# cszheng-ioa/Sixty-years-of-frequency-domain-monaural-speech-enhancement

Hardware: AMD Instinct MI355X
Metric: utterances/sec, 16 kHz 4 s clips, DCCRN decode (STFT->network->iSTFT) (higher is better)
Workload: dtype f32; 1 GPU; BASELINE configs[2]: DCCRN complex-mask, compressed input (0.5/2.0), 16 kHz x 4 s clips, batch 256 per MI355X, utterance-sharded; batch_per_gpu=256, global_batch=256, clip_samples=64000, parallelism=utterance shard x1 + RCCL gather to rank 0

## Files before the change

sixty-years-of-frequency-domain-monaural-speech-enhancement_amd/csrc/gemmconv.h:

```cpp
#pragma once
#include <hip/hip_runtime.h>
#include <vector>

namespace se {

constexpr int GC_MAX_TAPS = 16;
constexpr int GC_MAX_ROWS = 8;
constexpr int GC_MAX_KCP = 48;
constexpr int GC_TAB_KOFF = GC_MAX_ROWS + 2 * GC_MAX_TAPS;
constexpr int gc_kcp_max(int BM) { return 32; }
constexpr int gc_bld_max(int BM) { return (BM >= 128 || BM <= 32) ? 9 : 13; }
constexpr int gc_blocks_per_cu(int BM) { return BM <= 32 ? 6 : 3; }

enum Act : int { ACT_NONE = 0, ACT_PRELU = 1, ACT_ELU = 2, ACT_SOFTPLUS = 3, ACT_SIGMOID = 4, ACT_TANH = 5, ACT_RELU = 6 };
enum Epi : int {
    EPI_ACT = 0,
    EPI_LSTM = 1,
    EPI_GLU = 2,
    EPI_ADD = 3,
    EPI_MUL = 4,
    EPI_CMB = 5,
};

constexpr int GC_THIN_NT = 8;
// ... 28 lines not shown
    int si, so, po;
    int ntaps, nrows, dtmin, Wp;
    int CI_C, KC, KCp, nchunks;
    int act, epi;
    int n_ttiles, n_mtiles, Z;
    int dbg;
    int first_step;
    int gru;
    unsigned long long* timing;
    const unsigned* desc4;
    int t_base;
    int tb_soft;
    int pw4;
    int causal;
    const int* tlen;
    int qt2, qq_off, Qt;
    int pair, po2, fo_lim;
    short tdf[GC_MAX_TAPS], tdt[GC_MAX_TAPS];
    int nbuf;
    int trim;
    const unsigned* desc;
    const int* tab;
    float* stats;
    long st_b, st_c, st_f;
    float* cstats;
    long cs_b, cs_f;
    float* fz;
    long fz_b, fz_c, fz_f, fz_im;
    long fz_s;
    const float* nrm0;
    const float* nrm1;
    int flat_upr;
    int flat_units;
};
constexpr int GC_NRM_MAXC = 128;
constexpr int GC_FLAT_NRM_ROWS = 2;

struct GCGeom {
    int* tab = nullptr;
    unsigned* desc = nullptr;
    unsigned* desc4 = nullptr;
};
struct GCTail {
    int BN = 0, Wp = 0;
    GCGeom g;
};

struct GCSmallGeom {
    int dfmin = 0, dfmax = 0, dtmin = 0, dtmax = 0;
};

struct GCPlan {
    GCParams p{};
    int BM = 128, BN = 128;
    int lookback = 0;
    double flop_scale = 1.0;
    float* dA = nullptr;
    float* dWs = nullptr;
    unsigned* dDesc = nullptr;
    unsigned* dDesc4 = nullptr;
    GCSmallGeom small;
    bool tail_split = false;
    GCTail tail[3];
    GCTail qt2;
    GCTail flat[2];
    int flat_uw = 0;
    int qt2_nrows = 0, qt2_qoff = 0;
// ... 4 lines not shown
    float* dPostScale = nullptr;
    float* dPostShift = nullptr;
};

struct TapSpec {
    int ntaps = 0;
    int df[GC_MAX_TAPS];
    int dt[GC_MAX_TAPS];
};

GCPlan gc_make_plan(int M, int Cin, const TapSpec& taps, const std::vector<float>& w_logical,
                    const std::vector<float>& bias, const std::vector<float>& slope, int act, int epi,
                    int si, int so, int po, int tout_hint, int z = 1, int C0split = -1);
void gc_free_plan(GCPlan& pl);

void gc_register_overread_range(const void* lo, size_t bytes);
void gc_unregister_overread_range(const void* lo);

bool gc_stats_supported(const GCPlan& pl);
bool gc_nrm_supported(const GCPlan& pl);
void gc_launch(const GCPlan& pl, GCParams p, hipStream_t stream);
bool gc_launch_thin_pair(const GCParams& p0, const GCParams& p1, hipStream_t stream);

enum GCFamily : int { GC_FAM_TILE = 0, GC_FAM_THIN = 1, GC_FAM_THIN_PAIR = 2, GC_FAM_DIRECT = 3, GC_FAM_DIRECT_LDS = 4 };
struct GCLaunchRec {
    int family = GC_FAM_TILE;
    int BM = 0, BN = 0;
    int flat_upr = 0, upt = 0;
    int flat_rows = 0;
    int qt2 = 0, nrm = 0, res = 0, trim = 0, stats = 0, ragged = 0;
    int flat_nrm_refused = 0;
    long nblk = 0;
    int epi = 0, gru = 0;
};
void gc_set_launch_log(std::vector<GCLaunchRec>* log);
int gc_flat_rows_spanned(int B, int upr, int upt);

}
```

sixty-years-of-frequency-domain-monaural-speech-enhancement_amd/csrc/gemmconv.hip:

```cpp
#include "gemmconv.h"
#include "common.h"
#include "fastmath.h"
#include <algorithm>
#include <cmath>
#include <cstring>
#include <mutex>
#include <type_traits>

namespace se {

typedef float floatx16 __attribute__((ext_vector_type(16)));
typedef float floatx4 __attribute__((ext_vector_type(4)));

template <int N, typename F>
__device__ __forceinline__ void static_for(F&& f) {
    if constexpr (N > 0) {
        static_for<N - 1>(f);
        f(std::integral_constant<int, N - 1>{});
    }
}

__device__ __forceinline__ float fsig_(float x) { return fm_sigmoid(x); }
__device__ __forceinline__ float ftanh_(float x) { return fm_tanh(x); }
__device__ __forceinline__ float act_apply(float v, int act, float slope) {
// ... 252 lines not shown
            const int f = q * p.si + tabl[tabl[GC_MAX_ROWS + kr_ - nk_cil * p.ntaps]];
            nk_ok = kr_ < p.KC && f >= 0 && f < p.Fin;
        }
        pb_cil = tid / p.nrows;
    }

    unsigned aoff[A_IT];
    static_for<A_IT>([&](auto I) {
        constexpr int i = decltype(I)::value;
        int idx = tid + i * 256;
        if (idx >= nA4) idx = nA4 - 1;
        aoff[i] = 4u * (unsigned)((idx / (BM / 4)) * p.Mp + (idx % (BM / 4)) * 4);
    });
    unsigned boff[NB];
    unsigned vbits = 0;
    unsigned fullbits = 0;

    floatx16 acc[TM][TN];
#pragma unroll
    for (int i = 0; i < TM; ++i)
#pragma unroll
        for (int j = 0; j < TN; ++j)
#pragma unroll
            for (int r = 0; r < 16; ++r) acc[i][j][r] = 0.f;

    const int wm = wave / WN, wn = (WN == 4 && BN >= 256) ? ((wave + ttile) & 3) : wave % WN;
    constexpr int WNT = WN >= 2 ? WN / 2 : 1;
    const int wq = (qt2 && WN >= 2) ? wn / WNT : 0;
    const int wt = (qt2 && WN >= 2) ? wn % WNT : wn;
    const int am = wm * (TM * 32) + l31;
    const int bn = FLAT ? wn * (TN * UW) + l31 : wq * p.qq_off + wt * (TN * 32) + l31;
    const int jact = FLAT ? max(0, min(TN, p.flat_units - u0 - wn * TN))
                          : (q + wq >= p.Q) ? 0 : max(0, min(TN, (p.Tout - t0 - wt * (TN * 32) + 31) >> 5));

    int gchunk = 0;
    int buf = 0;

#define GC_MAKE_DESC(LIM)                                                                          \
    {                                                                                              \
        const int lim_ = (LIM);                                                                    \
        vbits = 0;                                                                                 \
         \
         \
         \
        unsigned dsc_[NB];                                                                         \
        {                                                                                          \
            const unsigned* __restrict__ dp_ = (pw4 ? p.desc4 : p.desc) + tid;                     \
            static_for<NB>([&](auto E) {                                                           \
                constexpr int e = decltype(E)::value;                                              \
                dsc_[e] = dp_[256 * e];                                                            \
            });                                                                                    \
        }                                                                                          \
        static_for<NB>([&](auto E) {                                                               \
            constexpr int e = decltype(E)::value;                                                  \
            const unsigned d_ = dsc_[e];                                                           \
            const int w = d_ & 0xfff, r = (d_ >> 12) & 0xf, cil = (d_ >> 16) & 0x7fff;             \
            const bool staged = (d_ >> 31) != 0;                                                   \
            const int f = q * p.si + tabl[staged ? r : 0];                                         \
             \
            const int uk_ = FLAT ? min(w / UW, UPT - 1) : 0;                                       \
            const int t = FLAT ? utab[4 * uk_ + 1] + p.dtmin + (w - uk_ * UW) : t0 + p.dtmin + w;  \
            const bool uok_ = !FLAT || utab[4 * uk_ + 2] != 0;                                     \
            const unsigned ub_ = (FLAT && uok_) ? (unsigned)utab[4 * uk_] * sb32 : 0u;             \
            const int fc = f < 0 ? 0 : (f >= p.Fin ? p.Fin - 1 : f);                               \
            const int tc = t < 0 ? 0 : (t >= p.Tin ? p.Tin - 1 : t);                               \
            const int cc = cil < lim_ ? cil : lim_ - 1;                                            \
// ... 115 lines not shown
        GC_WAIT_CHUNK();
        GC_TRIM_TAIL(buf);
        GC_T(3);
        __syncthreads();
        GC_T(4);

        for (int c = 0; c < nch; ++c) {
            if constexpr (RES) {
                if (c > 0 && buf == nbuf) {
                    __syncthreads();
                    for (int c2 = c; c2 < min(nch, c + nbuf); ++c2) {
                        if (c2 + 1 == nch && tail != p.CI_C) GC_MAKE_DESC(tail);
                        GC_LOAD_CHUNK(c2, c2 - c);
                    }
                    GC_WAIT_CHUNK();
                    __syncthreads();
                    buf = 0;
                }
            }
            if (!RES && c + 1 < nch && !(p.dbg & 1)) {
                if (__builtin_expect(c + 2 == nch && tail != p.CI_C, 0)) GC_MAKE_DESC(tail);
                GC_LOAD_CHUNK(c + 1, buf ^ 1);
            }
            GC_T(1);
            const float* Ab = As + buf * As_sz + hi * BM + am;
            const float* Bb = Bs + buf * Bs_sz + bn;
            const floatx4* nkb = nrmK + buf * (NRMB * KCP_MAX) + hi;
            int nkd[FLAT && NRM ? TN : 1];
            if constexpr (FLAT && NRM) {
#pragma unroll
                for (int j = 0; j < TN; ++j) nkd[j] = utab[4 * min(wn * TN + j, UPT - 1)] * KCP_MAX;
            }
            const int npair = p.KCp >> 1;
#define GC_FETCH(KP, AR, BR)                                                                       \
    {                                                                                              \
        int o_;                                                                                    \
        if constexpr (KOFF_REGS) o_ = koffv[(KP) < NPAIR ? (KP) : NPAIR - 1];                      \
        else o_ = koff_lds[2 * (KP) + hi];                                                         \
        _Pragma("unroll") for (int i = 0; i < TM; ++i) AR[i] = Ab[(2 * (KP)) * BM + i * 32];       \
        _Pragma("unroll") for (int j = 0; j < JN; ++j) BR[j] = Bb[o_ + j * UW];                    \
        if constexpr (NRM && !FLAT) {                                                              \
            const floatx4 pr_ = nkb[2 * (KP)];                                                     \
            _Pragma("unroll") for (int j = 0; j < JN; ++j) {                                       \
                const float t_ = fmaf(BR[j], pr_[0], pr_[1]);                                      \
                BR[j] = fmaf(fminf(t_, 0.f), pr_[2], t_);                                          \
            }                                                                                      \
        }                                                                                          \
        if constexpr (NRM && FLAT) {                                                               \
            _Pragma("unroll") for (int j = 0; j < JN; ++j) {                                       \
                const floatx4 pr_ = nkb[2 * (KP) + nkd[j]];                                        \
                const float t_ = fmaf(BR[j], pr_[0], pr_[1]);                                      \
                BR[j] = fmaf(fminf(t_, 0.f), pr_[2], t_);                                          \
            }                                                                                      \
        }                                                                                          \
    }
#define GC_MMA(AR, BR)                                                                             \
    _Pragma("unroll") for (int i = 0; i < TM; ++i)                                                 \
        _Pragma("unroll") for (int j = 0; j < JN; ++j)                                             \
            acc[i][j] = __builtin_amdgcn_mfma_f32_32x32x2f32(AR[i], BR[j], acc[i][j], 0, 0, 0);
            auto mma_chunk = [&](auto JN_) {
                constexpr int JN = decltype(JN_)::value;
                float ax[TM], bx[JN], ay[TM], by[JN];
                GC_FETCH(0, ax, bx);
                static_for<NPAIR / 2>([&](auto KP2) {
                    constexpr int kp = 2 * decltype(KP2)::value;
                    int np_ = npair;
                    asm volatile("" : "+s"(np_));
                    if (kp < np_) {
                        constexpr int NDS = (TM + 1) / 2 + (JN + 1) / 2 + (NRM ? (FLAT ? JN : 1) : 0);
                        GC_FETCH(kp + 1, ay, by);
                        __builtin_amdgcn_sched_group_barrier(0x100, NDS, 0);
                        GC_MMA(ax, bx);
                        __builtin_amdgcn_sched_group_barrier(0x008, TM * JN, 0);
                        if constexpr (NRM) __builtin_amdgcn_sched_group_barrier(0x002, 3 * JN, 0);
                        GC_FETCH(kp + 2, ax, bx);
                        __builtin_amdgcn_sched_group_barrier(0x100, NDS, 0);
                        GC_MMA(ay, by);
                        __builtin_amdgcn_sched_group_barrier(0x008, TM * JN, 0);
                        if constexpr (NRM) __builtin_amdgcn_sched_group_barrier(0x002, 3 * JN, 0);
                    }
                });
            };
            if (!(p.dbg & 4)) {
                if (jact == 1 && TN == 2) mma_chunk(std::integral_constant<int, 1>{});
                else if (jact >= 1) mma_chunk(std::integral_constant<int, TN>{});
            }
#undef GC_FETCH
#undef GC_MMA
            GC_T(2);
            if constexpr (RES) {
                buf += 1;
            } else {
                GC_WAIT_CHUNK();
                GC_TRIM_TAIL(buf ^ 1);
                GC_T(3);
                __syncthreads();
                GC_T(4);
                buf ^= 1;
            }
        }
        if constexpr (RES) __syncthreads();
// ... 557 lines not shown
                    v = act_apply(v, p.act, p.slope ? p.slope[j] : 0.f);
                    if (p.pair) {
                        const int cls = (2 * j) / p.pair, fo2 = (q0 + qq) * p.so + (cls ? p.po2 : p.po);
                        if (fo2 < p.fo_lim) dst[(long)(fo2 - fo) * p.d_f + (long)(j - cls * (p.pair >> 1)) * p.d_c + t] = v;
                    } else {
                        dst[(long)j * p.d_c + t] = v;
                    }
                }
            }
            continue;
        }
#pragma unroll
        for (int m = 0; m < MM; ++m) {
            if (m < p.M) {
                float v = acc[qq][m] + (bias ? bias[m] : 0.f);
                v = act_apply(v, p.act, p.slope ? p.slope[m] : 0.f);
                if (EPI == EPI_ADD) v += res[(long)m * p.x_c + t];
                if (EPI == EPI_MUL) v *= res[(long)m * p.x_c + t];
                if (EPI == EPI_ACT && p.pair) {
                    const int cls = m / p.pair, fo2 = (q0 + qq) * p.so + (cls ? p.po2 : p.po);
                    if (fo2 < p.fo_lim) dst[(long)(fo2 - fo) * p.d_f + (long)(m - cls * p.pair) * p.d_c + t] = v;
                    continue;
                }
                dst[(long)m * p.d_c + t] = v;
            }
        }
    }
}

template <int EPI, int NT>
__device__ __forceinline__ void gc_thin_body(const GCParams& p, const int blk) {
    constexpr int RB = 8, KG = 32, UN = 8;
    __shared__ float part[KG][RB][NT + 1];
    __shared__ int s_df[GC_MAX_TAPS], s_dt[GC_MAX_TAPS];
    const int tid = threadIdx.x, mi = tid & (RB - 1), kg = tid / RB;
#pragma unroll
    for (int j = 0; j < GC_MAX_TAPS; ++j)
        if (tid == j) {
            s_df[j] = p.tdf[j];
            s_dt[j] = p.tdt[j];
        }
    __syncthreads();
    const int nm = (p.M + RB - 1) / RB;
    const int mt = blk % nm;
    const int rest = blk / nm;
    const int q = rest % p.Q, b = rest / p.Q;
    const int m = mt * RB + mi, t0 = p.t_base, n = p.Tout - p.t_base;
    const int ntaps = p.ntaps, Ktot = (p.C0 + p.C1) * ntaps;
    const int nch0 = p.C0 > 0 ? (p.C0 + p.CI_C - 1) / p.CI_C : 0;
    float acc[NT];
#pragma unroll
    for (int t = 0; t < NT; ++t) acc[t] = 0.f;
    for (int k0 = kg; k0 < Ktot; k0 += KG * UN) {
        float w[UN], xv[UN][NT];
#pragma unroll
        for (int u = 0; u < UN; ++u) {
            const int kk = k0 + u * KG;
            const bool kok = kk < Ktot;
            const int kc = kok ? kk : 0;
            const int ci = kc / ntaps, j = kc - ci * ntaps;
            const bool seg = ci >= p.C0;
            const int cs = seg ? ci - p.C0 : ci;
            const int chunk = (seg ? nch0 : 0) + cs / p.CI_C, cil = cs % p.CI_C;
            const float wv = p.A[((long)chunk * p.KCp + cil * ntaps + j) * p.Mp + m];
            const int f = q * p.si + s_df[j];
            const bool fok = kok && f >= 0 && f < p.Fin;
            const int fc = fok ? f : 0;
            const float* __restrict__ src = seg ? p.src1 + (long)b * p.s1_b + (long)cs * p.s1_c + (long)fc * p.s1_f
                                                : p.src0 + (long)b * p.s0_b + (long)cs * p.s0_c + (long)fc * p.s0_f;
            const int tb = t0 + s_dt[j];
            w[u] = fok ? wv : 0.f;
#pragma unroll
            for (int t = 0; t < NT; ++t) {
                const int ti = tb + t;
                const bool ok = t < n && ti >= 0 && ti < p.Tin;
                const float x = src[ok ? ti : 0];
                xv[u][t] = ok ? x : 0.f;
            }
        }
#pragma unroll
        for (int u = 0; u < UN; ++u)
#pragma unroll
            for (int t = 0; t < NT; ++t) acc[t] = fmaf(w[u], xv[u][t], acc[t]);
    }
#pragma unroll
    for (int t = 0; t < NT; ++t) part[kg][mi][t] = acc[t];
    __syncthreads();
    const bool fold = tid < RB * NT;
    const int r = tid & (RB - 1), t = (tid / RB) & (NT - 1);
    float tot = 0.f;
    if (fold) {
#pragma unroll
        for (int g = 0; g < KG; ++g) tot += part[g][r][t];
    }
    __syncthreads();
    if (fold) part[0][r][t] = tot;
    __syncthreads();
// ... 54 lines not shown
__global__ __launch_bounds__(256) void gc_thin_pair_kernel(const GCThinPair a) {
    const int cls = (int)blockIdx.x >= a.nblk0 ? 1 : 0;
    gc_thin_body<EPI, NT>(a.p[cls], (int)blockIdx.x - (cls ? a.nblk0 : 0));
}
template <int EPI>
static void gc_thin_launch_n(const GCParams& p, dim3 grid, int n, hipStream_t stream) {
    if (n <= 1) hipLaunchKernelGGL((gc_thin_kernel<EPI, 1>), grid, dim3(256), 0, stream, p);
    else if (n <= 2) hipLaunchKernelGGL((gc_thin_kernel<EPI, 2>), grid, dim3(256), 0, stream, p);
    else if (n <= 4) hipLaunchKernelGGL((gc_thin_kernel<EPI, 4>), grid, dim3(256), 0, stream, p);
    else hipLaunchKernelGGL((gc_thin_kernel<EPI, 8>), grid, dim3(256), 0, stream, p);
}
static thread_local std::vector<GCLaunchRec>* g_launch_log = nullptr;
static thread_local int g_flat_nrm_refused = 0;
void gc_set_launch_log(std::vector<GCLaunchRec>* log) { g_launch_log = log; }
static void gc_log_launch(int family, const GCParams& p, long nblk, int BM = 0, int BN = 0, bool res = false) {
    if (!g_launch_log) return;
    GCLaunchRec r;
    r.family = family;
    r.BM = BM;
    r.BN = BN;
    r.flat_upr = p.flat_upr;
    r.upt = p.flat_upr ? BN / 32 : 0;
    r.flat_rows = p.flat_upr ? gc_flat_rows_spanned(p.B, p.flat_upr, BN / 32) : 0;
    r.qt2 = p.qt2;
    r.nrm = (p.nrm0 || p.nrm1) ? 1 : 0;
    r.res = res ? 1 : 0;
    r.trim = p.trim;
    r.stats = (p.stats || p.cstats) ? 1 : 0;
    r.ragged = p.tlen ? 1 : 0;
    r.flat_nrm_refused = g_flat_nrm_refused;
    r.nblk = nblk;
    r.epi = p.epi;
    r.gru = p.gru;
    g_launch_log->push_back(r);
}
int gc_flat_rows_spanned(int B, int upr, int upt) {
    const long units = (long)B * upr, tiles = (units + upt - 1) / upt;
    int most = 0;
    for (long k = 0; k < std::min<long>(tiles, upr); ++k) {
        const long u0 = k * upt, u1 = std::min(u0 + upt, units) - 1;
        most = std::max(most, (int)(u1 / upr - u0 / upr + 1));
    }
    return most;
}

constexpr long GC_THIN_MAX_BLOCKS = 8192;
static long gc_thin_blocks(const GCParams& p) {
    const int n = p.Tout - p.t_base;
    if ((p.Ws && p.pair) || n > GC_THIN_NT || p.Z > 1 || p.stats || p.cstats || p.nrm0 || p.nrm1) return 0;
    if (p.epi != EPI_ACT && p.epi != EPI_ADD && p.epi != EPI_MUL && p.epi != EPI_GLU && p.epi != EPI_LSTM) return 0;
    if (p.epi == EPI_LSTM && (p.M & 3)) return 0;
    const long nblk = (long)((p.M + 7) >> 3) * p.Q * p.B;
    if (nblk > GC_THIN_MAX_BLOCKS) return 0;
    if (!p.Ws) {
        const int nt = n <= 1 ? 1 : (n <= 2 ? 2 : (n <= 4 ? 4 : 8));
        const double waves_thin = std::ceil((double)nblk / 2048.0);
        const double waves_mfma = std::ceil((double)std::max(p.Z, 1) * p.B * p.Q * std::max(p.n_mtiles, 1) / 512.0);
        if ((long)p.B * n > 64 || nblk > 2800 * waves_mfma || waves_thin * (1 + nt) > 12 * waves_mfma) return 0;
    }
    return nblk;
}
static bool gc_thin_launch(const GCParams& p, hipStream_t stream) {
    const long nblk = (p.fz || p.dst_elu) ? 0 : gc_thin_blocks(p);
    if (nblk <= 0) return false;
    const int n = p.Tout - p.t_base;
    dim3 grid((unsigned)nblk);
// ... 62 lines not shown
            case EPI_GLU:
                if constexpr (MM >= 2) gc_small_lds_launch<MM, EPI_GLU>(p, grid, shm, CC, NR, sg, stream);
                break;
            default: SE_CHECK(false, "direct small-M path: unsupported epilogue");
        }
        SE_HIP(hipGetLastError());
        gc_log_launch(GC_FAM_DIRECT_LDS, p, nblk8);
        return;
    }
    const long nblk = (long)((p.Tout + 255) / 256) * p.Q * p.B * p.Z;
    SE_CHECK(nblk > 0 && nblk < (1L << 31), "grid size");
    dim3 grid((unsigned)nblk);
    switch (p.epi) {
        case EPI_ACT: hipLaunchKernelGGL((gc_small_kernel<MM, EPI_ACT>), grid, dim3(256), 0, stream, p); break;
        case EPI_ADD: hipLaunchKernelGGL((gc_small_kernel<MM, EPI_ADD>), grid, dim3(256), 0, stream, p); break;
        case EPI_MUL: hipLaunchKernelGGL((gc_small_kernel<MM, EPI_MUL>), grid, dim3(256), 0, stream, p); break;
        case EPI_GLU:
            if constexpr (MM >= 2) hipLaunchKernelGGL((gc_small_kernel<MM, EPI_GLU>), grid, dim3(256), 0, stream, p);
            break;
        default: SE_CHECK(false, "direct small-M path: unsupported epilogue");
    }
    SE_HIP(hipGetLastError());
    gc_log_launch(GC_FAM_DIRECT, p, nblk);
}

static size_t gc_lds_bytes(const GCParams& p, int BM, size_t epi_bytes, int nbuf = 2) {
    const size_t as = (size_t)((p.KCp * (BM / 4) + 255) / 256) * 1024, bs = (size_t)((p.CI_C * p.nrows * p.Wp + 255) / 256) * 256;
    const size_t nrb = p.flat_upr ? GC_FLAT_NRM_ROWS : 1;
    const size_t nrm = ((p.nrm0 || p.nrm1) ? (size_t)(nrb * GC_NRM_MAXC + 2 * nrb * gc_kcp_max(BM) + 2) * 16 : 0) + (p.flat_upr ? 128 : 0);
    const size_t cst = p.cstats ? (size_t)4 * 256 * 2 * 4 : 0;
    return std::max((size_t)nbuf * (as + bs) * 4, epi_bytes + cst) + (GC_TAB_KOFF + GC_MAX_KCP + 8) * 4 + (size_t)4 * BM * 4 + 64 + nrm;
}

GCGeom gc_build_geom(const TapSpec& taps, const std::vector<int>& rows, int dtmin, int nrows, int Wp, int cic, int KC, int NB) {
    GCGeom g;
    std::vector<int> tab(GC_TAB_KOFF + GC_MAX_KCP + 8, 0);
    for (int r = 0; r < nrows; ++r) tab[r] = rows[r];
    for (int j = 0; j < taps.ntaps; ++j) {
        tab[GC_MAX_ROWS + j] = (int)(std::find(rows.begin(), rows.end(), taps.df[j]) - rows.begin());
        tab[GC_MAX_ROWS + GC_MAX_TAPS + j] = taps.dt[j];
    }
    for (int k = 0; k < KC; ++k) {
        const int cil = k / taps.ntaps, j = k - cil * taps.ntaps;
        tab[GC_TAB_KOFF + k] = cil * (nrows * Wp) + tab[GC_MAX_ROWS + j] * Wp + (taps.dt[j] - dtmin);
    }
    SE_HIP(hipMalloc(&g.tab, tab.size() * sizeof(int)));
    SE_HIP(hipMemcpy(g.tab, tab.data(), tab.size() * sizeof(int), hipMemcpyHostToDevice));
    const int npatch = cic * nrows * Wp, gpr = Wp / 4;
    SE_CHECK(Wp % 4 == 0 && Wp < 4096 && nrows <= 16 && cic < 32768, "patch descriptor field overflow");
    std::vector<unsigned> desc((size_t)NB * 256, 0u), d4((size_t)NB * 256, 0u);
    for (int e = 0; e < NB; ++e)
        for (int t = 0; t < 256; ++t) {
            const int fe = t + 256 * e;
            if (fe < npatch) {
                const int rr = fe / Wp, w = fe - rr * Wp, cil = rr / nrows, r = rr - cil * nrows;
                desc[(size_t)e * 256 + t] = (unsigned)w | ((unsigned)r << 12) | ((unsigned)cil << 16) | 0x80000000u;
            }
            if (4 * fe < npatch) {
                const int rr = fe / gpr, w = 4 * (fe - rr * gpr), cil = rr / nrows, r = rr - cil * nrows;
                d4[(size_t)e * 256 + t] = (unsigned)w | ((unsigned)r << 12) | ((unsigned)cil << 16) | 0x80000000u;
            }
        }
    SE_HIP(hipMalloc(&g.desc, desc.size() * sizeof(unsigned)));
    SE_HIP(hipMemcpy(g.desc, desc.data(), desc.size() * sizeof(unsigned), hipMemcpyHostToDevice));
    SE_HIP(hipMalloc(&g.desc4, d4.size() * sizeof(unsigned)));
    SE_HIP(hipMemcpy(g.desc4, d4.data(), d4.size() * sizeof(unsigned), hipMemcpyHostToDevice));
    return g;
}

GCPlan gc_make_plan(int M, int Cin, const TapSpec& taps, const std::vector<float>& w, const std::vector<float>& bias,
                    const std::vector<float>& slope, int act, int epi, int si, int so, int po, int tout_hint, int Z,
                    int C0split) {
    const int C0 = (C0split < 0 || C0split > Cin) ? Cin : C0split;
    SE_CHECK(taps.ntaps >= 1 && taps.ntaps <= GC_MAX_TAPS, "tap count");
    SE_CHECK((long)w.size() == (long)Z * M * Cin * taps.ntaps, "weight size mismatch in gc_make_plan");
    GCPlan pl;
    GCParams& p = pl.p;
    pl.BM = M >= 96 ? 128 : (M >= 48 ? 64 : 32);
// ... 17 lines not shown
        SE_CHECK(taps.df[j] >= -32768 && taps.df[j] <= 32767 && taps.dt[j] >= -32768 && taps.dt[j] <= 32767, "tap offset range");
        p.tdf[j] = (short)taps.df[j];
        p.tdt[j] = (short)taps.dt[j];
    }
    p.causal = dtmax <= 0;
    pl.lookback = std::max(-dtmin, 0);
    dtmin = -((std::max(-dtmin, 0) + 3) & ~3);
    dtmax = (std::max(dtmax, 0) + 3) & ~3;
    p.dtmin = dtmin;
    p.Wp = pl.BN + (dtmax - dtmin);
    SE_CHECK(p.nrows * p.Wp <= gc_bld_max(pl.BM) * 256, "tap span too wide for one staged patch");
    int cic = 1;
    double best = -1.0;
    for (int c = 1; c <= std::max(std::max(C0, Cin - C0), 1); ++c) {
        const int kc = c * taps.ntaps, kcp = (kc + 3) & ~3;
        const bool pw = taps.ntaps == 1;
        const int kmax = pw ? (pl.BM >= 128 ? 24 : 32) : gc_kcp_max(pl.BM);
        const int cap = gc_bld_max(pl.BM) * 256 * (pw ? 4 : 1);
        if (kcp > kmax || c * p.nrows * p.Wp > cap) continue;
        if (pl.BM == 64 && pl.BN == 128 && taps.ntaps > 1 && epi != EPI_LSTM && kc > 12 &&
            (long)c * p.nrows * (256 + (dtmax - dtmin)) > 4608)
            continue;
        const double score = (double)kc / kcp + 1e-4 * kc;
        if (score > best) {
            best = score;
            cic = c;
        }
    }
    p.CI_C = cic;
    p.KC = cic * taps.ntaps;
    p.KCp = (p.KC + 3) & ~3;
    SE_CHECK(p.KCp <= gc_kcp_max(pl.BM), "single-channel chunk exceeds K budget");
    {
        GCGeom g = gc_build_geom(taps, rows, dtmin, p.nrows, p.Wp, cic, p.KC, gc_bld_max(pl.BM));
        pl.dTab = g.tab;
        pl.dDesc = g.desc;
        pl.dDesc4 = g.desc4;
        p.tab = g.tab;
        p.desc = g.desc;
        p.desc4 = g.desc4;
        pl.tail_split = taps.ntaps != 1;
        if (pl.BN == 128 && pl.BM == 128) {
            pl.tail[0].BN = 32;
            pl.tail[0].Wp = 32 + (dtmax - dtmin);
            pl.tail[0].g = gc_build_geom(taps, rows, dtmin, p.nrows, pl.tail[0].Wp, cic, p.KC, gc_bld_max(pl.BM));
        }
        if (pl.BN == 128 && epi != EPI_LSTM && taps.ntaps > 1) {
            std::vector<int> r2 = rows;
            for (int r : rows)
                if (std::find(r2.begin(), r2.end(), r + si) == r2.end()) r2.push_back(r + si);
            std::sort(r2.begin(), r2.end());
            const bool interval = r2.back() - r2.front() + 1 == (int)r2.size();
            const int wp2 = 64 + (dtmax - dtmin);
            if (interval && (int)r2.size() <= GC_MAX_ROWS && (int)r2.size() < 2 * p.nrows &&
                cic * (int)r2.size() * wp2 <= gc_bld_max(pl.BM) * 256) {
                pl.qt2.BN = 64;
                pl.qt2.Wp = wp2;
                pl.qt2.g = gc_build_geom(taps, r2, dtmin, (int)r2.size(), wp2, cic, p.KC, gc_bld_max(pl.BM));
                pl.qt2_nrows = (int)r2.size();
                pl.qt2_qoff = si * wp2;
            }
        }
        if (pl.BN == 128 && pl.BM == 64 && epi != EPI_LSTM && taps.ntaps > 1) {
            pl.tail[2].BN = 256;
            pl.tail[2].Wp = 256 + (dtmax - dtmin);
            pl.tail[2].g = gc_build_geom(taps, rows, dtmin, p.nrows, pl.tail[2].Wp, cic, p.KC, gc_bld_max(pl.BM));
        }
        static const int wide128_env = getenv("SE_GC_WIDE128") ? atoi(getenv("SE_GC_WIDE128")) : 1;
        if (wide128_env && pl.BN == 128 && pl.BM == 128 && taps.ntaps == 1 && epi == EPI_LSTM && cic * 256 <= 6 * 1024) {
            pl.tail[2].BN = 256;
            pl.tail[2].Wp = 256;
            pl.tail[2].g = gc_build_geom(taps, rows, dtmin, p.nrows, 256, cic, p.KC, gc_bld_max(pl.BM));
        }
        static const int flat_env = getenv("SE_GC_FLAT") ? atoi(getenv("SE_GC_FLAT")) : 1;
        if (flat_env && pl.BM == 64 && pl.BN == 128 && epi != EPI_LSTM && p.causal && dtmin >= -4 && Z == 1) {
            const int uw = 32 - dtmin;
            pl.flat_uw = uw;
            const int nbk = gc_bld_max(pl.BM);
            if ((long)cic * p.nrows * 4 * uw <= (long)nbk * 256 * 4) {
                pl.flat[0].BN = 128;
                pl.flat[0].Wp = 4 * uw;
                pl.flat[0].g = gc_build_geom(taps, rows, dtmin, p.nrows, 4 * uw, cic, p.KC, nbk);
            }
            if (pl.BM == 64 && (long)cic * p.nrows * 8 * uw <= 4608) {
                pl.flat[1].BN = 256;
                pl.flat[1].Wp = 8 * uw;
                pl.flat[1].g = gc_build_geom(taps, rows, dtmin, p.nrows, 8 * uw, cic, p.KC, nbk);
            }
        }
        if (pl.BN == 128 && (pl.BM == 64 || pl.BM == 128) && epi != EPI_LSTM) {
            pl.tail[1].BN = 64;
            pl.tail[1].Wp = 64 + (dtmax - dtmin);
            pl.tail[1].g = gc_build_geom(taps, rows, dtmin, p.nrows, pl.tail[1].Wp, cic, p.KC, gc_bld_max(pl.BM));
        }
    }
    const int nch0 = (C0 + cic - 1) / cic, nch1 = (Cin - C0 + cic - 1) / cic;
    p.nchunks = nch0 + nch1;
    p.M = M;
    p.Mp = ((M + pl.BM - 1) / pl.BM) * pl.BM;
    p.n_mtiles = p.Mp / pl.BM;
    p.act = act;
    p.epi = epi;
    p.si = si;
    p.so = so;
    p.po = po;
    p.Z = Z;
    p.C0 = C0;
    p.C1 = Cin - C0;
    const size_t per_z = (size_t)std::max(p.nchunks, 1) * p.KCp * p.Mp;
    std::vector<float> packed(per_z * Z, 0.f);
    for (int z = 0; z < Z; ++z)
        for (int m = 0; m < M; ++m)
            for (int ci = 0; ci < Cin; ++ci)
                for (int j = 0; j < taps.ntaps; ++j) {
                    const int cs = ci < C0 ? ci : ci - C0;
                    const int chunk = (ci < C0 ? 0 : nch0) + cs / cic, cil = cs % cic;
                    const size_t dst = z * per_z + ((size_t)chunk * p.KCp + (cil * taps.ntaps + j)) * p.Mp + m;
                    packed[dst] = w[(((size_t)z * M + m) * Cin + ci) * taps.ntaps + j];
                }
    p.A_z = (long)per_z;
    pl.dA = to_device(packed);
    p.A = pl.dA;
    if (M <= 4 && (epi == EPI_ACT || epi == EPI_ADD || epi == EPI_MUL || (epi == EPI_GLU && M % 2 == 0))) {
        const int MM = M <= 1 ? 1 : (M <= 2 ? 2 : 4);
        std::vector<float> ws((size_t)Z * Cin * taps.ntaps * MM, 0.f);
        for (int z = 0; z < Z; ++z)
            for (int m = 0; m < M; ++m)
                for (int ci = 0; ci < Cin; ++ci)
                    for (int j = 0; j < taps.ntaps; ++j)
                        ws[(((size_t)z * Cin + ci) * taps.ntaps + j) * MM + m] = w[(((size_t)z * M + m) * Cin + ci) * taps.ntaps + j];
        pl.dWs = to_device(ws);
        p.Ws = pl.dWs;
        pl.small.dfmin = pl.small.dfmax = taps.df[0];
        pl.small.dtmin = pl.small.dtmax = taps.dt[0];
        for (int j = 1; j < taps.ntaps; ++j) {
            pl.small.dfmin = std::min(pl.small.dfmin, taps.df[j]);
            pl.small.dfmax = std::max(pl.small.dfmax, taps.df[j]);
            pl.small.dtmin = std::min(pl.small.dtmin, taps.dt[j]);
            pl.small.dtmax = std::max(pl.small.dtmax, taps.dt[j]);
        }
    }
    if (!bias.empty()) {
        SE_CHECK((long)bias.size() == (long)Z * M, "bias size");
        pl.dBias = to_device(bias);
        p.bias = pl.dBias;
        p.bias_z = M;
    }
    if (!slope.empty()) {
        SE_CHECK((long)slope.size() == M, "slope size");
        pl.dSlope = to_device(slope);
// ... 76 lines not shown
}
static bool gc_flat_supported(int BM, int BN, int epi, int uw) {
    switch (epi) {
        case EPI_ACT: return gc_flat_inst(BM, BN, EPI_ACT, uw);
        case EPI_ADD: return gc_flat_inst(BM, BN, EPI_ADD, uw);
        case EPI_GLU: return gc_flat_inst(BM, BN, EPI_GLU, uw);
        case EPI_CMB: return gc_flat_inst(BM, BN, EPI_CMB, uw);
        default: return false;
    }
}
template <int BM, int BN, int WM, int WN, int EPI, bool NRMv, int UWv>
static void gc_launch_flat_k(const GCParams& p, long nblk, size_t lds, hipStream_t stream) {
    static bool attr_fl[64] = {};
    if (first_on_device(attr_fl)) {
        SE_HIP(hipFuncSetAttribute(reinterpret_cast<const void*>(&gc_kernel<BM, BN, WM, WN, EPI, false, false, false, NRMv, UWv>),
                                   hipFuncAttributeMaxDynamicSharedMemorySize, 160 * 1024));
    }
    hipLaunchKernelGGL((gc_kernel<BM, BN, WM, WN, EPI, false, false, false, NRMv, UWv>), dim3((unsigned)nblk), dim3(256), lds, stream, p);
    SE_HIP(hipGetLastError());
    gc_log_launch(GC_FAM_TILE, p, nblk, BM, BN);
}

template <int BM, int BN, int WM, int WN, int EPI, bool RES = false>
static void gc_launch_e(const GCParams& p_in, hipStream_t stream) {
    const size_t epi = (size_t)(4 * (BM / WM) * 36) * sizeof(float);
    const size_t lds = gc_lds_bytes(p_in, BM, epi, RES ? p_in.nbuf : 2);
    static bool attr_set[64] = {};
    if (first_on_device(attr_set)) {
        SE_HIP(hipFuncSetAttribute(reinterpret_cast<const void*>(&gc_kernel<BM, BN, WM, WN, EPI, RES>),
                                   hipFuncAttributeMaxDynamicSharedMemorySize, 160 * 1024));
    }
    const long nblk = (long)p_in.Z * (p_in.flat_upr ? 1 : p_in.B) * p_in.Qt * p_in.n_ttiles * p_in.n_mtiles;
    SE_CHECK(nblk > 0 && nblk < (1L << 31), "grid size");
    const GCParams& p = p_in;
    if (p.flat_upr) {
        const int uw = p.Wp / (BN / 32);
        SE_CHECK(!RES && !p.fz && !p.trim && !p.qt2 && p.pw4 && p.t_base == 0, "gc_launch: flattened tiles on a launch they do not cover");
        const bool nrm = p.nrm0 || p.nrm1;
        if constexpr (!RES && gc_flat_inst(BM, BN, EPI, 36)) {
            if (uw == 36) {
                if constexpr (EPI == EPI_ACT && BM == 64) {
                    if (nrm) {
                        SE_CHECK(p.causal && p.Z == 1 && p.C0 + p.C1 <= GC_NRM_MAXC, "gc_launch: on-the-fly InstanceNorm needs causal taps and <= 128 input channels");
                        SE_CHECK(gc_flat_rows_spanned(p.B, p.flat_upr, BN / 32) <= GC_FLAT_NRM_ROWS,
                                 "gc_launch: a flattened tile with on-the-fly InstanceNorm would span more batch rows than it holds parameters for");
                        gc_launch_flat_k<BM, BN, WM, WN, EPI, true, 36>(p, nblk, lds, stream);
                        return;
                    }
                }
                SE_CHECK(!nrm, "gc_launch: this flattened variant cannot normalise its sources on the fly");
                gc_launch_flat_k<BM, BN, WM, WN, EPI, false, 36>(p, nblk, lds, stream);
                return;
            }
        }
        if constexpr (!RES && gc_flat_inst(BM, BN, EPI, 32)) {
            if (uw == 32) {
                if constexpr (EPI == EPI_ACT && BM == 64) {
                    if (nrm) {
                        SE_CHECK(p.causal && p.Z == 1 && p.C0 + p.C1 <= GC_NRM_MAXC, "gc_launch: on-the-fly InstanceNorm needs causal taps and <= 128 input channels");
                        SE_CHECK(gc_flat_rows_spanned(p.B, p.flat_upr, BN / 32) <= GC_FLAT_NRM_ROWS,
                                 "gc_launch: a flattened tile with on-the-fly InstanceNorm would span more batch rows than it holds parameters for");
                        gc_launch_flat_k<BM, BN, WM, WN, EPI, true, 32>(p, nblk, lds, stream);
                        return;
                    }
                }
                SE_CHECK(!nrm, "gc_launch: this flattened variant cannot normalise its sources on the fly");
                gc_launch_flat_k<BM, BN, WM, WN, EPI, false, 32>(p, nblk, lds, stream);
// ... 78 lines not shown
    if (nblk > 256 || nb <= 2 || p.Tout - p.t_base > 64) return false;
    const size_t epi = (size_t)(4 * BM_div_WM * 36) * sizeof(float);
    while (nb > 2 && gc_lds_bytes(p, BM, epi, nb) > 158 * 1024) --nb;
    if (nb <= 2) return false;
    p.nbuf = nb;
    return true;
}

bool gc_nrm_supported(const GCPlan& pl) {
    static const bool on = !(getenv("SE_IN_FOLD") && atoi(getenv("SE_IN_FOLD")) == 0);
    return on && !pl.p.Ws && pl.p.epi == EPI_ACT && pl.BM == 64 && pl.p.causal && pl.p.Z == 1 && pl.p.C0 + pl.p.C1 <= GC_NRM_MAXC;
}

bool gc_stats_supported(const GCPlan& pl) {
    return !pl.p.Ws && (pl.p.epi == EPI_GLU || (pl.p.epi == EPI_ACT && pl.BM == 64));
}

void gc_launch(const GCPlan& pl, GCParams p, hipStream_t stream) {
    SE_CHECK(p.C0 == pl.p.C0 && p.C1 == pl.p.C1, "gc_launch: source channel split differs from the plan");
    SE_CHECK(!p.dst_elu || (p.epi == EPI_GLU && p.Z == 1), "gc_launch: the second (ELU) store belongs to the gated epilogue");
    if (p.epi == EPI_LSTM && p.first_step && p.C1 == 0) p.C0 = 0;
    g_flat_nrm_refused = 0;
    if (p.t_base > 0 && gc_thin_launch(p, stream)) return;
    if (p.tb_soft) p.t_base &= ~3;
    const int tb = p.t_base, Tspan = p.Tout - tb;
    SE_CHECK(tb >= 0 && (tb & 3) == 0 && Tspan > 0, "gc_launch: first output frame must be a multiple of 4 below Tout");
    SE_CHECK(tb == 0 || (!p.stats && !p.cstats), "gc_launch: the statistics epilogue needs whole rows");
    p.n_ttiles = (Tspan + pl.BN - 1) / pl.BN;
    p.Qt = p.Q;
    p.qt2 = 0;
    p.qq_off = 0;
    static const int dbg_env = getenv("SE_GC_DBG") ? atoi(getenv("SE_GC_DBG")) : 0;
    p.dbg = dbg_env;
    SE_CHECK((double)p.CI_C * (double)std::max(p.s0_c, p.s1_c) + (double)p.Fin * (double)std::max(p.s0_f, p.s1_f) + p.Tin < 1.0e9,
             "gc_launch: source plane too large for 32-bit patch byte offsets");
    constexpr long trim_min = 8192;
    const bool trim_ok = p.epi == EPI_ACT && (long)p.Z * p.B * p.Q * p.n_ttiles * p.n_mtiles >= trim_min;
    p.pw4 = (p.desc4 && (p.Tin % 4 == 0 || ((p.causal || trim_ok) && gc_overread_ok(p.src0) && gc_overread_ok(p.src1)))) ? 1 : 0;
    p.trim = (p.pw4 && !p.causal && p.Tin % 4 != 0) ? 1 : 0;
    SE_CHECK(!p.stats || gc_stats_supported(pl), "gc_launch: this tile configuration has no statistics epilogue");
    SE_CHECK(!p.cstats || (gc_stats_supported(pl) && p.n_mtiles == 1 && p.Z == 1),
             "gc_launch: column statistics need a statistics tile configuration and one m-tile (M " + std::to_string(p.M) + ", BM " +
                 std::to_string(pl.BM) + ", m-tiles " + std::to_string(p.n_mtiles) + ", epilogue " + std::to_string(p.epi) + ", direct " +
                 std::to_string(p.Ws != nullptr) + ")");
    SE_CHECK(p.pw4 || p.CI_C * p.nrows * p.Wp <= gc_bld_max(pl.BM) * 256,
             "pointwise layer with a row length that is not a multiple of 4 needs its sources inside the engine arena");
    if (gc_thin_launch(p, stream)) return;
    if (p.Ws) {
        SE_CHECK(!p.fz, "gc_launch: the direct (<= 4 channel) path cannot fold the branch interaction into its store");
        SE_CHECK(!p.dst_elu, "gc_launch: the direct (<= 4 channel) path has no second (ELU) store");
        SE_CHECK(!p.nrm0 && !p.nrm1, "gc_launch: the direct (<= 4 channel) path cannot normalise its sources on the fly");
        if (p.M <= 1) gc_small_launch<1>(p, pl.small, stream);
        else if (p.M <= 2) gc_small_launch<2>(p, pl.small, stream);
        else gc_small_launch<4>(p, pl.small, stream);
        return;
    }
    {
        const GCTail& alt = pl.tail[1];
        const long nblk = (long)p.Z * p.B * p.Q * p.n_ttiles * p.n_mtiles;
        static const int alt_n64 = getenv("SE_GC_ALT_N64") ? atoi(getenv("SE_GC_ALT_N64")) : 4096;
        if (alt.BN == 64 && nblk < (pl.BM == 64 ? alt_n64 : 256)) {
            GCParams pa = p;
            pa.n_ttiles = (Tspan + 63) / 64;
            pa.Wp = alt.Wp;
            pa.tab = alt.g.tab;
            pa.desc = alt.g.desc;
// ... 140 lines not shown
```

Measured before the change: 2715 utt/s.

## Reorder packed conv weights frequency-major and skip out-of-plane K rows

Packs each chunk's weight K rows grouped by frequency offset (kfm layout) when the tap set forms a full frequency x time rectangle, and rebuilds the patch offset tables to match. Tile blocks then compute the range of frequency rows that fall inside [0, Fin) for their output bin and run the MFMA K loop only over that contiguous range. This skips multiply work on zero-padded frequency edges for layers with few output bins (Q <= 8). It adds per-block range setup, a non-zero starting fetch, and a new weight layout that the thin path must also follow.

```diff
diff --git a/sixty-years-of-frequency-domain-monaural-speech-enhancement_amd/csrc/gemmconv.h b/sixty-years-of-frequency-domain-monaural-speech-enhancement_amd/csrc/gemmconv.h
--- a/sixty-years-of-frequency-domain-monaural-speech-enhancement_amd/csrc/gemmconv.h
+++ b/sixty-years-of-frequency-domain-monaural-speech-enhancement_amd/csrc/gemmconv.h
@@ -84,7 +84,13 @@
     const float* nrm1;
     int flat_upr;
     int flat_units;
+    int kfm;
+    int ndf;
+    short kdf[GC_MAX_ROWS];
+    short tkb[GC_MAX_TAPS];
+    int inplane;
 };
+constexpr int GC_INPLANE_MAXQ = 8;
 constexpr int GC_NRM_MAXC = 128;
 constexpr int GC_FLAT_NRM_ROWS = 2;
 
@@ -155,6 +161,8 @@
     int flat_nrm_refused = 0;
     long nblk = 0;
     int epi = 0, gru = 0;
+    int kfm = 0;
+    int inplane = 0;
 };
 void gc_set_launch_log(std::vector<GCLaunchRec>* log);
 int gc_flat_rows_spanned(int B, int upr, int upt);
diff --git a/sixty-years-of-frequency-domain-monaural-speech-enhancement_amd/csrc/gemmconv.hip b/sixty-years-of-frequency-domain-monaural-speech-enhancement_amd/csrc/gemmconv.hip
--- a/sixty-years-of-frequency-domain-monaural-speech-enhancement_amd/csrc/gemmconv.hip
+++ b/sixty-years-of-frequency-domain-monaural-speech-enhancement_amd/csrc/gemmconv.hip
@@ -308,6 +308,26 @@
     const int bn = FLAT ? wn * (TN * UW) + l31 : wq * p.qq_off + wt * (TN * 32) + l31;
     const int jact = FLAT ? max(0, min(TN, p.flat_units - u0 - wn * TN))
                           : (q + wq >= p.Q) ? 0 : max(0, min(TN, (p.Tout - t0 - wt * (TN * 32) + 31) >> 5));
+
+    constexpr bool INPL = !RES && !FZ && !NRM && !FLAT && EPI != EPI_LSTM;
+    int lo_w = 0, hi_w = p.KCp >> 1;
+    if constexpr (INPL) {
+        if (p.inplane) {
+            const int fq = (q + wq) * p.si;
+            int jl = 0, jh = 0;
+#pragma unroll
+            for (int j = 0; j < GC_MAX_ROWS; ++j) {
+                const int f = fq + p.kdf[j];
+                if (j < p.ndf) {
+                    jl += f < 0 ? 1 : 0;
+                    jh += f < p.Fin ? 1 : 0;
+                }
+            }
+            const int ppt = (p.CI_C * p.kfm) >> 1;
+            lo_w = __builtin_amdgcn_readfirstlane(jl * ppt);
+            hi_w = __builtin_amdgcn_readfirstlane(max(jh, jl) * ppt);
+        }
+    }
 
     int gchunk = 0;
     int buf = 0;
@@ -489,6 +509,8 @@
                 for (int j = 0; j < TN; ++j) nkd[j] = utab[4 * min(wn * TN + j, UPT - 1)] * KCP_MAX;
             }
             const int npair = p.KCp >> 1;
+            const bool whole = !INPL || (c + 1 == nch && tail != p.CI_C);
+            const int lo_c = whole ? 0 : lo_w, hi_c = whole ? npair : hi_w;
 #define GC_FETCH(KP, AR, BR)                                                                       \
     {                                                                                              \
         int o_;                                                                                    \
@@ -518,12 +540,18 @@
             auto mma_chunk = [&](auto JN_) {
                 constexpr int JN = decltype(JN_)::value;
                 float ax[TM], bx[JN], ay[TM], by[JN];
-                GC_FETCH(0, ax, bx);
+                if (!INPL || lo_c == 0) {
+                    GC_FETCH(0, ax, bx);
+                } else {
+                    const int o_ = koff_lds[2 * lo_c + hi];
+                    _Pragma("unroll") for (int i = 0; i < TM; ++i) ax[i] = Ab[(2 * lo_c) * BM + i * 32];
+                    _Pragma("unroll") for (int j = 0; j < JN; ++j) bx[j] = Bb[o_ + j * UW];
+                }
                 static_for<NPAIR / 2>([&](auto KP2) {
                     constexpr int kp = 2 * decltype(KP2)::value;
-                    int np_ = npair;
+                    int np_ = INPL ? lo_c : npair;
                     asm volatile("" : "+s"(np_));
-                    if (kp < np_) {
+                    if (INPL ? (unsigned)(kp - np_) < (unsigned)(hi_c - lo_c) : kp < np_) {
                         constexpr int NDS = (TM + 1) / 2 + (JN + 1) / 2 + (NRM ? (FLAT ? JN : 1) : 0);
                         GC_FETCH(kp + 1, ay, by);
                         __builtin_amdgcn_sched_group_barrier(0x100, NDS, 0);
@@ -1147,13 +1175,14 @@
 __device__ __forceinline__ void gc_thin_body(const GCParams& p, const int blk) {
     constexpr int RB = 8, KG = 32, UN = 8;
     __shared__ float part[KG][RB][NT + 1];
-    __shared__ int s_df[GC_MAX_TAPS], s_dt[GC_MAX_TAPS];
+    __shared__ int s_df[GC_MAX_TAPS], s_dt[GC_MAX_TAPS], s_kb[GC_MAX_TAPS];
     const int tid = threadIdx.x, mi = tid & (RB - 1), kg = tid / RB;
 #pragma unroll
     for (int j = 0; j < GC_MAX_TAPS; ++j)
         if (tid == j) {
             s_df[j] = p.tdf[j];
             s_dt[j] = p.tdt[j];
+            s_kb[j] = p.tkb[j];
         }
     __syncthreads();
     const int nm = (p.M + RB - 1) / RB;
@@ -1177,7 +1206,8 @@
             const bool seg = ci >= p.C0;
             const int cs = seg ? ci - p.C0 : ci;
             const int chunk = (seg ? nch0 : 0) + cs / p.CI_C, cil = cs % p.CI_C;
-            const float wv = p.A[((long)chunk * p.KCp + cil * ntaps + j) * p.Mp + m];
+            const int kr = p.kfm ? s_kb[j] + cil * p.kfm : cil * ntaps + j;
+            const float wv = p.A[((long)chunk * p.KCp + kr) * p.Mp + m];
             const int f = q * p.si + s_df[j];
             const bool fok = kok && f >= 0 && f < p.Fin;
             const int fc = fok ? f : 0;
@@ -1298,6 +1328,8 @@
     r.nblk = nblk;
     r.epi = p.epi;
     r.gru = p.gru;
+    r.kfm = p.kfm;
+    r.inplane = (family == GC_FAM_TILE) ? p.inplane : 0;
     g_launch_log->push_back(r);
 }
 int gc_flat_rows_spanned(int B, int upr, int upt) {
@@ -1426,7 +1458,9 @@
     return std::max((size_t)nbuf * (as + bs) * 4, epi_bytes + cst) + (GC_TAB_KOFF + GC_MAX_KCP + 8) * 4 + (size_t)4 * BM * 4 + 64 + nrm;
 }
 
-GCGeom gc_build_geom(const TapSpec& taps, const std::vector<int>& rows, int dtmin, int nrows, int Wp, int cic, int KC, int NB) {
+static inline int gc_krow(const GCParams& kp, int ntaps, int cil, int j) { return kp.kfm ? kp.tkb[j] + cil * kp.kfm : cil * ntaps + j; }
+GCGeom gc_build_geom(const TapSpec& taps, const std::vector<int>& rows, int dtmin, int nrows, int Wp, int cic, int KC, int NB,
+                     const GCParams& kp) {
     GCGeom g;
     std::vector<int> tab(GC_TAB_KOFF + GC_MAX_KCP + 8, 0);
     for (int r = 0; r < nrows; ++r) tab[r] = rows[r];
@@ -1434,10 +1468,10 @@
         tab[GC_MAX_ROWS + j] = (int)(std::find(rows.begin(), rows.end(), taps.df[j]) - rows.begin());
         tab[GC_MAX_ROWS + GC_MAX_TAPS + j] = taps.dt[j];
     }
-    for (int k = 0; k < KC; ++k) {
-        const int cil = k / taps.ntaps, j = k - cil * taps.ntaps;
-        tab[GC_TAB_KOFF + k] = cil * (nrows * Wp) + tab[GC_MAX_ROWS + j] * Wp + (taps.dt[j] - dtmin);
-    }
+    for (int cil = 0; cil < cic; ++cil)
+        for (int j = 0; j < taps.ntaps; ++j)
+            tab[GC_TAB_KOFF + gc_krow(kp, taps.ntaps, cil, j)] = cil * (nrows * Wp) + tab[GC_MAX_ROWS + j] * Wp + (taps.dt[j] - dtmin);
+    SE_CHECK(KC == cic * taps.ntaps, "gc_build_geom: K rows of a chunk");
     SE_HIP(hipMalloc(&g.tab, tab.size() * sizeof(int)));
     SE_HIP(hipMemcpy(g.tab, tab.data(), tab.size() * sizeof(int), hipMemcpyHostToDevice));
     const int npatch = cic * nrows * Wp, gpr = Wp / 4;
@@ -1521,7 +1555,34 @@
     p.KCp = (p.KC + 3) & ~3;
     SE_CHECK(p.KCp <= gc_kcp_max(pl.BM), "single-channel chunk exceeds K budget");
     {
-        GCGeom g = gc_build_geom(taps, rows, dtmin, p.nrows, p.Wp, cic, p.KC, gc_bld_max(pl.BM));
+        std::vector<int> dts;
+        for (int j = 0; j < taps.ntaps; ++j)
+            if (std::find(dts.begin(), dts.end(), taps.dt[j]) == dts.end()) dts.push_back(taps.dt[j]);
+        std::sort(dts.begin(), dts.end());
+        const int ndf = p.nrows, ndt = (int)dts.size();
+        bool rect = ndf * ndt == taps.ntaps;
+        std::vector<char> seen((size_t)ndf * ndt, 0);
+        for (int j = 0; j < taps.ntaps && rect; ++j) {
+            const int a = (int)(std::find(rows.begin(), rows.end(), taps.df[j]) - rows.begin());
+            const int b = (int)(std::find(dts.begin(), dts.end(), taps.dt[j]) - dts.begin());
+            if (seen[(size_t)a * ndt + b]) rect = false;
+            seen[(size_t)a * ndt + b] = 1;
+        }
+        const bool nrm_form = epi == EPI_ACT && pl.BM == 64 && p.causal && Z == 1 && Cin <= GC_NRM_MAXC;
+        const bool flat_form = pl.BM == 64 && pl.BN == 128 && p.causal && dtmin >= -4 && Z == 1;
+        p.ndf = ndf;
+        for (int r = 0; r < ndf; ++r) p.kdf[r] = (short)rows[r];
+        if (ndf >= 2 && rect && (cic * ndt) % 4 == 0 && !nrm_form && !flat_form && epi != EPI_LSTM && M > 4) {
+            p.kfm = ndt;
+            for (int j = 0; j < taps.ntaps; ++j) {
+                const int a = (int)(std::find(rows.begin(), rows.end(), taps.df[j]) - rows.begin());
+                const int b = (int)(std::find(dts.begin(), dts.end(), taps.dt[j]) - dts.begin());
+                p.tkb[j] = (short)(a * cic * ndt + b);
+            }
+        }
+    }
+    {
+        GCGeom g = gc_build_geom(taps, rows, dtmin, p.nrows, p.Wp, cic, p.KC, gc_bld_max(pl.BM), p);
         pl.dTab = g.tab;
         pl.dDesc = g.desc;
         pl.dDesc4 = g.desc4;
@@ -1532,7 +1593,7 @@
         if (pl.BN == 128 && pl.BM == 128) {
             pl.tail[0].BN = 32;
             pl.tail[0].Wp = 32 + (dtmax - dtmin);
-            pl.tail[0].g = gc_build_geom(taps, rows, dtmin, p.nrows, pl.tail[0].Wp, cic, p.KC, gc_bld_max(pl.BM));
+            pl.tail[0].g = gc_build_geom(taps, rows, dtmin, p.nrows, pl.tail[0].Wp, cic, p.KC, gc_bld_max(pl.BM), p);
         }
         if (pl.BN == 128 && epi != EPI_LSTM && taps.ntaps > 1) {
             std::vector<int> r2 = rows;
@@ -1545,7 +1606,7 @@
                 cic * (int)r2.size() * wp2 <= gc_bld_max(pl.BM) * 256) {
                 pl.qt2.BN = 64;
                 pl.qt2.Wp = wp2;
-                pl.qt2.g = gc_build_geom(taps, r2, dtmin, (int)r2.size(), wp2, cic, p.KC, gc_bld_max(pl.BM));
+                pl.qt2.g = gc_build_geom(taps, r2, dtmin, (int)r2.size(), wp2, cic, p.KC, gc_bld_max(pl.BM), p);
                 pl.qt2_nrows = (int)r2.size();
                 pl.qt2_qoff = si * wp2;
             }
@@ -1553,13 +1614,13 @@
         if (pl.BN == 128 && pl.BM == 64 && epi != EPI_LSTM && taps.ntaps > 1) {
             pl.tail[2].BN = 256;
             pl.tail[2].Wp = 256 + (dtmax - dtmin);
-            pl.tail[2].g = gc_build_geom(taps, rows, dtmin, p.nrows, pl.tail[2].Wp, cic, p.KC, gc_bld_max(pl.BM));
+            pl.tail[2].g = gc_build_geom(taps, rows, dtmin, p.nrows, pl.tail[2].Wp, cic, p.KC, gc_bld_max(pl.BM), p);
         }
         static const int wide128_env = getenv("SE_GC_WIDE128") ? atoi(getenv("SE_GC_WIDE128")) : 1;
         if (wide128_env && pl.BN == 128 && pl.BM == 128 && taps.ntaps == 1 && epi == EPI_LSTM && cic * 256 <= 6 * 1024) {
             pl.tail[2].BN = 256;
             pl.tail[2].Wp = 256;
-            pl.tail[2].g = gc_build_geom(taps, rows, dtmin, p.nrows, 256, cic, p.KC, gc_bld_max(pl.BM));
+            pl.tail[2].g = gc_build_geom(taps, rows, dtmin, p.nrows, 256, cic, p.KC, gc_bld_max(pl.BM), p);
         }
         static const int flat_env = getenv("SE_GC_FLAT") ? atoi(getenv("SE_GC_FLAT")) : 1;
         if (flat_env && pl.BM == 64 && pl.BN == 128 && epi != EPI_LSTM && p.causal && dtmin >= -4 && Z == 1) {
@@ -1569,18 +1630,18 @@
             if ((long)cic * p.nrows * 4 * uw <= (long)nbk * 256 * 4) {
                 pl.flat[0].BN = 128;
                 pl.flat[0].Wp = 4 * uw;
-                pl.flat[0].g = gc_build_geom(taps, rows, dtmin, p.nrows, 4 * uw, cic, p.KC, nbk);
+                pl.flat[0].g = gc_build_geom(taps, rows, dtmin, p.nrows, 4 * uw, cic, p.KC, nbk, p);
             }
             if (pl.BM == 64 && (long)cic * p.nrows * 8 * uw <= 4608) {
                 pl.flat[1].BN = 256;
                 pl.flat[1].Wp = 8 * uw;
-                pl.flat[1].g = gc_build_geom(taps, rows, dtmin, p.nrows, 8 * uw, cic, p.KC, nbk);
+                pl.flat[1].g = gc_build_geom(taps, rows, dtmin, p.nrows, 8 * uw, cic, p.KC, nbk, p);
             }
         }
         if (pl.BN == 128 && (pl.BM == 64 || pl.BM == 128) && epi != EPI_LSTM) {
             pl.tail[1].BN = 64;
             pl.tail[1].Wp = 64 + (dtmax - dtmin);
-            pl.tail[1].g = gc_build_geom(taps, rows, dtmin, p.nrows, pl.tail[1].Wp, cic, p.KC, gc_bld_max(pl.BM));
+            pl.tail[1].g = gc_build_geom(taps, rows, dtmin, p.nrows, pl.tail[1].Wp, cic, p.KC, gc_bld_max(pl.BM), p);
         }
     }
     const int nch0 = (C0 + cic - 1) / cic, nch1 = (Cin - C0 + cic - 1) / cic;
@@ -1604,7 +1665,7 @@
                 for (int j = 0; j < taps.ntaps; ++j) {
                     const int cs = ci < C0 ? ci : ci - C0;
                     const int chunk = (ci < C0 ? 0 : nch0) + cs / cic, cil = cs % cic;
-                    const size_t dst = z * per_z + ((size_t)chunk * p.KCp + (cil * taps.ntaps + j)) * p.Mp + m;
+                    const size_t dst = z * per_z + ((size_t)chunk * p.KCp + gc_krow(p, taps.ntaps, cil, j)) * p.Mp + m;
                     packed[dst] = w[(((size_t)z * M + m) * Cin + ci) * taps.ntaps + j];
                 }
     p.A_z = (long)per_z;
@@ -1747,7 +1808,8 @@
     }
     const long nblk = (long)p_in.Z * (p_in.flat_upr ? 1 : p_in.B) * p_in.Qt * p_in.n_ttiles * p_in.n_mtiles;
     SE_CHECK(nblk > 0 && nblk < (1L << 31), "grid size");
-    const GCParams& p = p_in;
+    GCParams p = p_in;
+    if (RES || EPI == EPI_LSTM || p.flat_upr || p.fz || p.nrm0 || p.nrm1) p.inplane = 0;
     if (p.flat_upr) {
         const int uw = p.Wp / (BN / 32);
         SE_CHECK(!RES && !p.fz && !p.trim && !p.qt2 && p.pw4 && p.t_base == 0, "gc_launch: flattened tiles on a launch they do not cover");
@@ -1892,6 +1954,8 @@
     p.qq_off = 0;
     static const int dbg_env = getenv("SE_GC_DBG") ? atoi(getenv("SE_GC_DBG")) : 0;
     p.dbg = dbg_env;
+    static const int inplane_env = getenv("SE_GC_INPLANE") ? atoi(getenv("SE_GC_INPLANE")) : 1;
+    p.inplane = (p.kfm && inplane_env && p.Q <= GC_INPLANE_MAXQ) ? 1 : 0;
     SE_CHECK((double)p.CI_C * (double)std::max(p.s0_c, p.s1_c) + (double)p.Fin * (double)std::max(p.s0_f, p.s1_f) + p.Tin < 1.0e9,
              "gc_launch: source plane too large for 32-bit patch byte offsets");
     constexpr long trim_min = 8192;
```

After: 2710 utt/s. About the same (-0.2%).
